# filrg/attackFL

Measured on AMD Instinct MI355X. Metric: FL rounds/sec (whole node) + test-acc, TransformerModel/ICU, 8 clients, higher is better.
Workload: dtype bf16; 1 GPU; model=TransformerModel, global_batch=1024, seq_len=1, parallelism=fl8-clients-over-1-ranks, clients=8, local_epochs=5, rows_per_client=12000-15000, mode=fedavg, trainer=fused

## Files before the change

### csrc/kernels/tf2.hip

```cpp
#include "common.h"
#include "kernels.h"
#include "tf_common.h"
#include "fused_common.h"
#define ONCHIP_NO_AGPR
#include "onchip.h"

using namespace tf;

namespace t2 {

using namespace oc;



constexpr int LDDN = 24 * 2, LDVO = LD64 + 16;
constexpr int B_IMG_D = 0;
constexpr int B_IMG_V = B_IMG_D + 64 * LDDN;
constexpr int B_IMG_O = B_IMG_V + 64 * LDVO;
constexpr int B_IMG_F1 = B_IMG_O + 64 * LDVO;
constexpr int B_IMG_F2 = B_IMG_F1 + 16 * LD64;
constexpr int B_H0 = B_IMG_F2 + 64 * LD32;
constexpr int B_A = B_H0 + 16384;
constexpr int B_X1N = B_A + 16384;
constexpr int B_DF3 = B_X1N + 16384;
constexpr int B_DO = B_DF3 + 16384;
constexpr int B_DV = B_DO + 16384;
constexpr int B_DZ0 = B_DV + 16384;
constexpr int B_XIN = B_DZ0 + 16384;
constexpr int B_F2 = B_XIN + 4096;
constexpr int B_DF0 = B_F2 + 4096;
constexpr int B_NVEC = 648;
constexpr int B_VEC = B_DF0 + 4096;
constexpr int B_NLN = 6 * 64;
constexpr int B_DBL = B_VEC + B_NVEC * 4;
constexpr int B_DBL_BYTES = B_NLN * 8;
constexpr int B_MISC = B_DBL + B_DBL_BYTES;
constexpr int B_CNT_A = B_MISC + 32;
constexpr int B_CNT_B = B_MISC + 36;
constexpr int B_CNT_C = B_MISC + 40;
constexpr int B_TOTAL = B_MISC + 64;
enum { VS_DB = 0, VS_VB, VS_OB, VS_G1, VS_B1, VS_F2B, VS_G2, VS_B2, VS_G3, VS_B3 };
constexpr int VS_F1B = 640;

#ifndef TF2_HLD1
#define TF2_HLD1 (LD128 + 16)
#endif
#ifndef TF2_HLD2
#define TF2_HLD2 (LD64 + 16)
#endif
constexpr int HLD1 = TF2_HLD1, HLD2 = TF2_HLD2;
constexpr int H_IMG_W1 = 0;
constexpr int H_IMG_W2 = H_IMG_W1 + 64 * HLD1;
constexpr int H_CAT = H_IMG_W2 + 32 * HLD2;
constexpr int H_A1 = H_CAT + 32768;
constexpr int H_DZ1 = H_A1 + 16384;
constexpr int H_DZ2 = H_DZ1 + 16384;
constexpr int H_NVEC = 132;
constexpr int H_VEC = H_DZ2 + 8192;
constexpr int H_PART = H_VEC + H_NVEC * 4;
constexpr int H_LOSS = H_PART + 8 * H_NVEC * 4;
constexpr int H_CNT = H_LOSS + 64;
constexpr int H_TOTAL = H_CNT + 16;
enum { HV_B1 = 0, HV_B2 = 64, HV_WO = 96, HV_BO = 128 };

constexpr int SMEM_CORE = B_TOTAL > H_TOTAL ? B_TOTAL : H_TOTAL;
// ... 19 lines not shown
  float s;
  const int f = colsum64(x, lane, s);
  lds_addq(smem + B_DBL, 64 * k + f, s);
}
__host__ __device__ constexpr int ln_seg(int k) { return k < 2 ? VS_G1 + k : VS_G2 + (k - 2); }
static_assert(ln_seg(0) == VS_G1 && ln_seg(1) == VS_B1 && ln_seg(2) == VS_G2 && ln_seg(3) == VS_B2 &&
              ln_seg(4) == VS_G3 && ln_seg(5) == VS_B3, "DBL order");

__device__ __forceinline__ uint32_t mask16(uint32_t key, uint32_t layer, int r, int g, uint32_t thr) {
  uint32_t m = 0;
#pragma unroll
  for (int t = 0; t < 4; ++t) {
#pragma unroll
    for (int h = 0; h < 2; ++h) {
      const uint32_t x = hash3(key, layer, (uint32_t)r, (uint32_t)(8 * t + 2 * g + h));
      m |= ((x & 0xFFFFu) >= thr ? 1u : 0u) << (4 * t + 2 * h);
      m |= ((x >> 16) >= thr ? 1u : 0u) << (4 * t + 2 * h + 1);
    }
  }
  return m;
}


#ifdef TF2_STAMPS
struct Stamp {
  bool on = false;
  int who = 0;
  uchar* smem = nullptr;
  __device__ __forceinline__ void operator()(int id, int tid) {
    if (!on) return;
    const uint64_t now = __builtin_amdgcn_s_memrealtime();
    if (tid == who) {
      LDS_AS uint64_t* t = (LDS_AS uint64_t*)(smem + ST_OFF);
      t[id] += now - t[ST_N - 1];
      t[ST_N - 1] = now;
    }
  }
};
#else
struct Stamp {
  __device__ __forceinline__ void operator()(int, int) {}
};
#endif

enum { ABL_U3 = 1, ABL_UADAM = 2, ABL_UDW = 4, ABL_COLSUM = 8, ABL_HEADUPD = 16, ABL_U1 = 32 };
#if defined(TF2_STAMPS) && defined(TF2_ABL)
#define ABL(K, b) ((TF2_ABL & (b)) != 0)
#else
#define ABL(K, b) false
#endif



#ifndef TF2_NO_PRIO
__device__ __forceinline__ void prio_hi() { __builtin_amdgcn_s_setprio(2); }
__device__ __forceinline__ void prio_lo() { __builtin_amdgcn_s_setprio(0); }
#else
__device__ __forceinline__ void prio_hi() {}
__device__ __forceinline__ void prio_lo() {}
#endif

template <int BR>
struct BrK {
  static constexpr BrOff o = BR == 0 ? OV : OL;
  static constexpr int din = BR == 0 ? D_V : D_L;
  static constexpr int xoff = BR == 0 ? 0 : D_V;
  static constexpr Mat MV{o.inproj_w + 128 * 64, 64, 64, B_IMG_V, LDVO};
  static constexpr Mat MO{o.out_w, 64, 64, B_IMG_O, LDVO};
  static __device__ __forceinline__ Mat vo(bool lo) {
    return Mat{lo ? MV.off : MO.off, 64, 64, lo ? B_IMG_V : B_IMG_O, LDVO};
  }
  static __device__ __forceinline__ int vec_param(int e) {
    if (e >= VS_F1B) return e - VS_F1B < FF ? o.ff0_b + (e - VS_F1B) : -1;
    const int s = e >> 6, i = e & 63;
    const int b = s == 0 ? o.dense_b : s == 1 ? o.inproj_b + 128 : s == 2 ? o.out_b : s == 3 ? o.ln1_w
                : s == 4 ? o.ln1_b : s == 5 ? o.ff3_b : s == 6 ? o.ln2_w : s == 7 ? o.ln2_b : s == 8 ? o.bn_w : o.bn_b;
    return b + i;
  }
};

struct Saved {
  uint32_t xh1[8], xh2[8], gp[8];
  float rstd1, rstd2;
  uint32_t m1, m2, matt;
  float gk[4];
};
__device__ __forceinline__ void save16(uint32_t (&d)[8], const float (&x)[16]) {
#pragma unroll
  for (int k = 0; k < 8; ++k) d[k] = pk2(x[2 * k], x[2 * k + 1]);
}
__device__ __forceinline__ void load16(float (&x)[16], const uint32_t (&d)[8]) {
#pragma unroll
  for (int k = 0; k < 8; ++k) {
    x[2 * k] = __uint_as_float(d[k] << 16);
    x[2 * k + 1] = __uint_as_float(d[k] & 0xFFFF0000u);
  }
}

constexpr int NCMP = 2;
struct BrState {
  VS cmp[NCMP];
};
__device__ __forceinline__ int vec_entry(int wave, int lane, int h) {
  const int w4 = wave & 3, g = lane >> 4, i16 = lane & 15;
  const bool lead = wave < 4;
  if (h == 0) {
    if (wave >= 2) return ln_seg(wave - 2) * 64 + lane;
    return wave == 0 && g == 0 && VS_F1B + i16 < B_NVEC ? VS_F1B + i16 : -1;
  }
  if (g < 2) return (w4 & 1) == 0 ? (lead ? VS_OB : VS_VB) * 64 + 16 * (2 * (w4 >> 1) + g) + i16 : -1;
  return lead ? (g == 2 ? VS_F2B : VS_DB) * 64 + 16 * w4 + i16 : -1;
}
__device__ __forceinline__ bool vec_real(int e) { return e >= 0 && e < VS_F1B + FF; }

template <int BR>
__device__ __forceinline__ void br_masks(uint32_t key, int r, int g, uint32_t& mk0, uint32_t& mk1) {
  const uint32_t ha = hash3(key, 8 * BR + L_ATT, r, 0), hb = hash3(key, 8 * BR + L_ATT, r, 1);
  const uint32_t matt = ((ha & 0xFFFFu) >= THR_P01 ? 1u : 0u) | ((ha >> 16) >= THR_P01 ? 2u : 0u) |
                        ((hb & 0xFFFFu) >= THR_P01 ? 4u : 0u) | ((hb >> 16) >= THR_P01 ? 8u : 0u);
  const uint32_t m1 = mask16(key, 8 * BR + L_D1, r, g, THR_P01), m2 = mask16(key, 8 * BR + L_D2, r, g, THR_P01);
  uint32_t kf = 0u;
  if (g < 2) {
    const uint32_t hd[2] = {hash3(key, 8 * BR + L_DF, r, 2 * g), hash3(key, 8 * BR + L_DF, r, 2 * g + 1)};
#pragma unroll
    for (int i = 0; i < 4; ++i) {
      const uint32_t u = (hd[i >> 1] >> ((i & 1) << 4)) & 0xFFFFu;
      kf |= (4 * g + i < FF && u >= THR_P01 ? 1u : 0u) << i;
    }
  }
  mk0 = m1 | (m2 << 16);
  mk1 = matt | (kf << 4);
}

template <int BR>
__device__ __forceinline__ void br_forward(uchar* smem, const float (&xin)[4], uint32_t mk0, uint32_t mk1, Saved& sv,
                                           u32x4 (&outp)[2], int lane, int wave) {
  using B = BrK<BR>;
  opq(lane, wave);
  const int g = lane >> 4, r = 16 * wave + (lane & 15);
  const uchar* vg = lane_vec(smem + B_VEC, g);
  st4<TK16>(smem + B_XIN, r, g, xin);
  float h0[16];
  sb();
  {
    const s4v bx = bfrag4(xin);
    f4v acc[4];
#pragma unroll
    for (int T = 0; T < 4; ++T)
      acc[T] = mma16(*(const LDS_AS s4v*)(smem + B_IMG_D + (16 * T + (lane & 15)) * LDDN + 8 * (lane >> 4)), bx, Z4);
    float bd[16], gp[16];
    vec16g(bd, vg + VS_DB * 256);
#pragma unroll
    for (int t = 0; t < 4; ++t)
#pragma unroll
      for (int i = 0; i < 4; i += 2) {
        gf2v g2;
        const gf2v y = gelu2(gf2v{acc[t][i] + bd[4 * t + i], acc[t][i + 1] + bd[4 * t + i + 1]}, g2);
        h0[4 * t + i] = y[0];
        h0[4 * t + i + 1] = y[1];
        gp[4 * t + i] = g2[0];
        gp[4 * t + i + 1] = g2[1];
      }
    save16(sv.gp, gp);
#pragma unroll
    for (int t = 0; t < 4; ++t) st4<TK64>(smem + B_H0, r, 4 * t + g, h0 + 4 * t);
  }
  float a[16];
  sb();
  {
    const s8v b0 = bfrag(h0, 0), b1 = bfrag(h0, 1);
    f4v acc[4];
#pragma unroll
    for (int T = 0; T < 4; ++T) {
      acc[T] = mma(wfrag(smem + B_IMG_V, LDVO, T, 0, lane), b0, Z4);
      acc[T] = mma(wfrag(smem + B_IMG_V, LDVO, T, 1, lane), b1, acc[T]);
    }
    sv.matt = mk1 & 0xFu;
    float bv[16];
    vec16g(bv, vg + VS_VB * 256);
#pragma unroll
    for (int t = 0; t < 4; ++t) {
      const float m = keepf(INV_K01, sv.matt, t);
#pragma unroll
      for (int i = 0; i < 4; ++i) a[4 * t + i] = (acc[t][i] + bv[4 * t + i]) * m;
    }
#pragma unroll
    for (int t = 0; t < 4; ++t) st4<TK64>(smem + B_A, r, 4 * t + g, a + 4 * t);
  }
  float x1n[16];
  sb();
  {
    const s8v b0 = bfrag(a, 0), b1 = bfrag(a, 1);
    f4v acc[4];
#pragma unroll
    for (int T = 0; T < 4; ++T) {
      acc[T] = mma(wfrag(smem + B_IMG_O, LDVO, T, 0, lane), b0, Z4);
      acc[T] = mma(wfrag(smem + B_IMG_O, LDVO, T, 1, lane), b1, acc[T]);
    }
    sv.m1 = mk0 & 0xFFFFu;
    float bo[16];
    vec16g(bo, vg + VS_OB * 256);
    float x1[16];
#pragma unroll
    for (int t = 0; t < 4; ++t)
#pragma unroll
      for (int i = 0; i < 4; ++i) {
        const int j = 4 * t + i;
        x1[j] = h0[j] + keepf((acc[t][i] + bo[j]) * INV_K01, sv.m1, j);
      }
    sv.rstd1 = ln_fwd2(x1);
    save16(sv.xh1, x1);
    float gm[16], bt[16];
    vec16g(gm, vg + VS_G1 * 256);
    vec16g(bt, vg + VS_B1 * 256);
    affine2(x1n, x1, gm, bt);
#pragma unroll
    for (int t = 0; t < 4; ++t) st4<TK64>(smem + B_X1N, r, 4 * t + g, x1n + 4 * t);
  }
  float f2v[4];
  sb();
  {
    f4v acc = mma(wfrag(smem + B_IMG_F1, LD64, 0, 0, lane), bfrag(x1n, 0), Z4);
    acc = mma(wfrag(smem + B_IMG_F1, LD64, 0, 1, lane), bfrag(x1n, 1), acc);
    const f4v bf = g < 2 ? *(const LDS_AS f4v*)(vg + VS_F1B * 4) : Z4;
#pragma unroll
    for (int i = 0; i < 4; ++i) {
      float gp;
      const float gl = gelu_and_grad(acc[i] + bf[i], gp);
      f2v[i] = keepf(gl * INV_K01, mk1, 4 + i);
      sv.gk[i] = keepf(gp * INV_K01, mk1, 4 + i);
    }
    st4<TK16>(smem + B_F2, r, g, f2v);
  }
  sb();
  {
    const s4v bf = bfrag4(f2v);
    f4v acc[4];
#pragma unroll
    for (int T = 0; T < 4; ++T) acc[T] = mma16(wfrag4(smem + B_IMG_F2, LD32, T, lane), bf, Z4);
    sv.m2 = mk0 >> 16;
    float b3[16];
    vec16g(b3, vg + VS_F2B * 256);
    float x2[16];
#pragma unroll
    for (int t = 0; t < 4; ++t)
#pragma unroll
      for (int i = 0; i < 4; ++i) {
        const int j = 4 * t + i;
        x2[j] = x1n[j] + keepf((acc[t][i] + b3[j]) * INV_K01, sv.m2, j);
      }
    sv.rstd2 = ln_fwd2(x2);
    save16(sv.xh2, x2);
    float gm[16], bt[16];
    vec16g(gm, vg + VS_G2 * 256);
    vec16g(bt, vg + VS_B2 * 256);
    affine2(x2, x2, gm, bt);
    ln_fwd2(x2);
    vec16g(gm, vg + VS_G3 * 256);
    vec16g(bt, vg + VS_B3 * 256);
    affine2(x2, x2, gm, bt);
    pack16(x2, outp);
  }
}

struct BwdPre {
  float xh3[16], rstd3;
  s8v f3[2];
};
__device__ __forceinline__ void br_bwd_pre(const uchar* smem, const Saved& sv, BwdPre& bp, int lane) {
  const uchar* vg = lane_vec(smem + B_VEC, lane >> 4);
  float gm[16], bt[16];
  load16(bp.xh3, sv.xh2);
  vec16g(gm, vg + VS_G2 * 256);
  vec16g(bt, vg + VS_B2 * 256);
  affine2(bp.xh3, bp.xh3, gm, bt);
  bp.rstd3 = ln_fwd2(bp.xh3);
#pragma unroll
  for (int j = 0; j < 16; ++j) asm volatile("" : "+v"(bp.xh3[j]));
  asm volatile("" : "+v"(bp.rstd3));
  bp.f3[0] = wtfrag<true>(smem + B_IMG_F2, LD32, 0, 0, lane);
  bp.f3[1] = wtfrag<true>(smem + B_IMG_F2, LD32, 0, 1, lane);
  asm volatile("" : "+v"(bp.f3[0]), "+v"(bp.f3[1]));
}

template <int BR>
__device__ __forceinline__ void br_backward(uchar* smem, const float (&dout)[16], const Saved& sv, const BwdPre& bp,
                                            const AdamK& K, int lane, int wave) {
  opq(lane, wave);
  const int g = lane >> 4, r = 16 * wave + (lane & 15);
  const uchar* vg = lane_vec(smem + B_VEC, g);
  float dr2[16];
  sb();
  {
    float gm[16], t[16], dx[16], xh[16];
#pragma unroll
    for (int j = 0; j < 16; ++j) xh[j] = bp.xh3[j];
    const float rstd3 = bp.rstd3;
#pragma unroll
    for (int j = 0; j < 16; ++j) t[j] = dout[j] * xh[j];
    if (!ABL(K, ABL_COLSUM)) ln_colsum(smem, 4, t, lane);
    if (!ABL(K, ABL_COLSUM)) ln_colsum(smem, 5, dout, lane);
    vec16g(gm, vg + VS_G3 * 256);
    ln_bwd2(dx, dout, xh, rstd3, gm);
    load16(xh, sv.xh2);
#pragma unroll
    for (int j = 0; j < 16; ++j) t[j] = dx[j] * xh[j];
    if (!ABL(K, ABL_COLSUM)) ln_colsum(smem, 2, t, lane);
    if (!ABL(K, ABL_COLSUM)) ln_colsum(smem, 3, dx, lane);
    vec16g(gm, vg + VS_G2 * 256);
    ln_bwd2(dr2, dx, xh, sv.rstd2, gm);
  }
  float df0[4];
  sb();
  {
    float d3[16];
#pragma unroll
    for (int j = 0; j < 16; ++j) d3[j] = keepf(dr2[j] * INV_K01, sv.m2, j);
#pragma unroll
    for (int t = 0; t < 4; ++t) st4<TK64>(smem + B_DF3, r, 4 * t + g, d3 + 4 * t);
    f4v acc = mma(bp.f3[0], bfrag(d3, 0), Z4);
    acc = mma(bp.f3[1], bfrag(d3, 1), acc);
#pragma unroll
    for (int i = 0; i < 4; ++i) df0[i] = acc[i] * sv.gk[i];
    st4<TK16>(smem + B_DF0, r, g, df0);
  }
  lds_signal(smem, B_CNT_C, lane);
  float dr1[16];
  sb();
  {
    const s4v bd = bfrag4(df0);
    float dx[16];
#pragma unroll
    for (int T = 0; T < 4; ++T) {
      const f4v acc = mma16(wtfrag4(smem + B_IMG_F1, LD64, T, lane), bd, Z4);
#pragma unroll
      for (int i = 0; i < 4; ++i) dx[4 * T + i] = acc[i] + dr2[4 * T + i];
    }
    float t[16], gm[16], xh[16];
    load16(xh, sv.xh1);
#pragma unroll
    for (int j = 0; j < 16; ++j) t[j] = dx[j] * xh[j];
    if (!ABL(K, ABL_COLSUM)) ln_colsum(smem, 0, t, lane);
    if (!ABL(K, ABL_COLSUM)) ln_colsum(smem, 1, dx, lane);
    vec16g(gm, vg + VS_G1 * 256);
    ln_bwd2(dr1, dx, xh, sv.rstd1, gm);
  }
  float dv[16];
  sb();
  {
    float dO[16];
#pragma unroll
    for (int j = 0; j < 16; ++j) dO[j] = keepf(dr1[j] * INV_K01, sv.m1, j);
#pragma unroll
    for (int t = 0; t < 4; ++t) st4<TK64>(smem + B_DO, r, 4 * t + g, dO + 4 * t);
    const s8v b0 = bfrag(dO, 0), b1 = bfrag(dO, 1);
#pragma unroll
    for (int T = 0; T < 4; ++T) {
      f4v acc = mma(wtfrag<true>(smem + B_IMG_O, LDVO, T, 0, lane), b0, Z4);
      acc = mma(wtfrag<true>(smem + B_IMG_O, LDVO, T, 1, lane), b1, acc);
      const float m = keepf(INV_K01, sv.matt, T);
#pragma unroll
      for (int i = 0; i < 4; ++i) dv[4 * T + i] = acc[i] * m;
    }
#pragma unroll
    for (int t = 0; t < 4; ++t) st4<TK64>(smem + B_DV, r, 4 * t + g, dv + 4 * t);
  }
  lds_signal(smem, B_CNT_A, lane);
  sb();
  {
    const s8v b0 = bfrag(dv, 0), b1 = bfrag(dv, 1);
    float dz[16], gp[16];
    load16(gp, sv.gp);
#pragma unroll
    for (int T = 0; T < 4; ++T) {
      f4v acc = mma(wtfrag<true>(smem + B_IMG_V, LDVO, T, 0, lane), b0, Z4);
      acc = mma(wtfrag<true>(smem + B_IMG_V, LDVO, T, 1, lane), b1, acc);
#pragma unroll
      for (int i = 0; i < 4; ++i) dz[4 * T + i] = (acc[i] + dr1[4 * T + i]) * gp[4 * T + i];
    }
#pragma unroll
    for (int t = 0; t < 4; ++t) st4<TK64>(smem + B_DZ0, r, 4 * t + g, dz + 4 * t);
  }
  lds_signal(smem, B_CNT_B, lane);
}


template <int BR>
__device__ __forceinline__ int cmp_param(int e) {
  return vec_real(e) ? BrK<BR>::vec_param(e) : -1;
}

__device__ __forceinline__ f4v unit_ld(__amdgpu_buffer_rsrc_t rm, int ui, int j, int lane) {
  return __builtin_bit_cast(f4v, __builtin_amdgcn_raw_buffer_load_b128(rm, (int)BR_UNITS + ((ui * 12 + j) * 64 + lane) * 16,
                                                                        0, 16));
}
__device__ __forceinline__ void unit_st(__amdgpu_buffer_rsrc_t rm, int ui, int j, int lane, f4v v) {
  __builtin_amdgcn_raw_buffer_store_b128(__builtin_bit_cast(u32x4, v), rm, (int)BR_UNITS + ((ui * 12 + j) * 64 + lane) * 16,
                                         0, 0);
  store_guard();
}
__device__ __forceinline__ void unit_adam(f4v (&U)[12], const f4v (&acc)[2][2], const AdamK& K) {
  float p[16], mm[16], vv[16], g[16], den[16];
#pragma unroll
  for (int t = 0; t < 4; ++t)
#pragma unroll
    for (int i = 0; i < 4; ++i) {
      mm[4 * t + i] = U[t][i];
      vv[4 * t + i] = U[4 + t][i];
      p[4 * t + i] = U[8 + t][i];
      g[4 * t + i] = acc[t >> 1][t & 1][i];
    }
#pragma unroll
  for (int e = 0; e < 16; ++e) {
    const float mk = mm[e] * K.keep;
    mm[e] = mk + K.c1 * (g[e] - mk);
    vv[e] = fk::B2 * vv[e] + (1.f - fk::B2) * g[e] * g[e];
  }
#pragma unroll
  for (int e = 0; e < 16; ++e) den[e] = __builtin_amdgcn_sqrtf(vv[e]);
#pragma unroll
  for (int e = 0; e < 16; ++e) den[e] = __builtin_amdgcn_rcpf(den[e] * K.rsqrt_bc2 + K.eps);
#pragma unroll
  for (int e = 0; e < 16; ++e) p[e] -= K.lr_bc1 * mm[e] * den[e];
#pragma unroll
  for (int t = 0; t < 4; ++t)
#pragma unroll
    for (int i = 0; i < 4; ++i) {
      U[t][i] = mm[4 * t + i];
      U[4 + t][i] = vv[4 * t + i];
      U[8 + t][i] = p[4 * t + i];
    }
}
__device__ __forceinline__ void unit_img(uchar* smem, const Mat& M, int Ta, int Tb, int lane, const u32x2v (&w)[4]) {
  const int i16 = lane & 15, g4 = 4 * (lane >> 4);
#pragma unroll
  for (int t = 0; t < 4; ++t)
    *(LDS_AS u32x2v*)(smem + M.img + (16 * (Tb + (t & 1)) + i16) * M.ld + pcol(16 * (Ta + (t >> 1)) + g4) * 2) = w[t];
}
__device__ __forceinline__ void unit_pack(const f4v (&U)[12], u32x2v (&w)[4]) {
#pragma unroll
  for (int t = 0; t < 4; ++t) w[t] = u32x2v{pk2(U[8 + t][0], U[8 + t][1]), pk2(U[8 + t][2], U[8 + t][3])};
}
__device__ __forceinline__ void unit_dw(const uchar* X, const uchar* DY, int Ta, int Tb, int lane, bool bias,
                                        f4v (&acc)[2][2], f4v (&bs)[2]) {
#pragma unroll
  for (int a = 0; a < 2; ++a)
#pragma unroll
    for (int b = 0; b < 2; ++b) acc[a][b] = Z4;
  bs[0] = bs[1] = Z4;
  uint32_t o1 = 0x3F803F80u;
  asm volatile("" : "+s"(o1));
  const s8v one = __builtin_bit_cast(s8v, u32x4{o1, o1, o1, o1});
#pragma unroll
  for (int s = 0; s < 4; ++s) {
    const s8v x0 = tfrag<TK64>(X, 32 * s, Ta, lane), x1 = tfrag<TK64>(X, 32 * s, Ta + 1, lane);
    const s8v y0 = tfrag<TK64>(DY, 32 * s, Tb, lane), y1 = tfrag<TK64>(DY, 32 * s, Tb + 1, lane);
    acc[0][0] = mma(x0, y0, acc[0][0]);
    acc[0][1] = mma(x0, y1, acc[0][1]);
    acc[1][0] = mma(x1, y0, acc[1][0]);
    acc[1][1] = mma(x1, y1, acc[1][1]);
    if (bias) {
      bs[0] = mma(one, y0, bs[0]);
      bs[1] = mma(one, y1, bs[1]);
    }
  }
}

__device__ __forceinline__ f4v smu_ld(__amdgpu_buffer_rsrc_t rm, int w4, int j, int lane) {
  return __builtin_bit_cast(f4v, __builtin_amdgcn_raw_buffer_load_b128(rm, (int)BR_SMALL + ((w4 * 9 + j) * 64 + lane) * 16,
                                                                        0, 16));
}
__device__ __forceinline__ void smu_st(__amdgpu_buffer_rsrc_t rm, int w4, int j, int lane, f4v v) {
  __builtin_amdgcn_raw_buffer_store_b128(__builtin_bit_cast(u32x4, v), rm, (int)BR_SMALL + ((w4 * 9 + j) * 64 + lane) * 16,
                                         0, 0);
  store_guard();
}
template <int BR>
__device__ __forceinline__ void smu_elem(int s, int w4, int lane, int i, int& pi, int& img) {
  using B = BrK<BR>;
  constexpr int din = BrK<BR>::din;
  const int g = lane >> 4, i16 = lane & 15;
  if (s == 0) {
    const int n = 16 * w4 + i16, k = 4 * g + i;
    pi = k < din ? B::o.dense_w + n * din + k : -1;
    img = B_IMG_D + n * LDDN + k * 2;
  } else if (s == 1) {
    const int n = 16 * w4 + i16, k = 4 * g + i;
    pi = k < FF ? B::o.ff3_w + n * FF + k : -1;
    img = B_IMG_F2 + n * LD32 + pcol(k) * 2;
  } else {
    const int n = i16, k = 16 * w4 + 4 * g + i;
    pi = n < FF ? B::o.ff0_w + n * 64 + k : -1;
    img = B_IMG_F1 + n * LD64 + pcol(k) * 2;
  }
}
__device__ __forceinline__ void smu_adam(f4v (&S)[9], const f4v (&gs)[3], const AdamK& K) {
  float p[12], mm[12], vv[12], g[12], den[12];
#pragma unroll
  for (int s = 0; s < 3; ++s)
#pragma unroll
    for (int i = 0; i < 4; ++i) {
      mm[4 * s + i] = S[s][i];
      vv[4 * s + i] = S[3 + s][i];
      p[4 * s + i] = S[6 + s][i];
      g[4 * s + i] = gs[s][i];
    }
#pragma unroll
  for (int e = 0; e < 12; ++e) {
    const float mk = mm[e] * K.keep;
    mm[e] = mk + K.c1 * (g[e] - mk);
    vv[e] = fk::B2 * vv[e] + (1.f - fk::B2) * g[e] * g[e];
  }
#pragma unroll
  for (int e = 0; e < 12; ++e) den[e] = __builtin_amdgcn_sqrtf(vv[e]);
#pragma unroll
  for (int e = 0; e < 12; ++e) den[e] = __builtin_amdgcn_rcpf(den[e] * K.rsqrt_bc2 + K.eps);
#pragma unroll
  for (int e = 0; e < 12; ++e) p[e] -= K.lr_bc1 * mm[e] * den[e];
#pragma unroll
  for (int s = 0; s < 3; ++s)
#pragma unroll
    for (int i = 0; i < 4; ++i) {
      S[s][i] = mm[4 * s + i];
      S[3 + s][i] = vv[4 * s + i];
      S[6 + s][i] = p[4 * s + i];
    }
}
template <int BR>
__device__ __forceinline__ void smu_img(uchar* smem, const f4v (&S)[9], int w4, int lane) {
#pragma unroll
  for (int s = 0; s < 3; ++s) {
    int pi, img;
    smu_elem<BR>(s, w4, lane, 0, pi, img);
    *(LDS_AS u32x2v*)(smem + img) = u32x2v{pk2(S[6 + s][0], S[6 + s][1]), pk2(S[6 + s][2], S[6 + s][3])};
  }
}

template <int N>
__device__ __forceinline__ void vec_adam(VS (&pa)[N], float (&m)[N], float (&v)[N], const float (&g)[N], float (&pn)[N],
                                         const AdamK& K) {
#pragma clang fp contract(off)
  float den[N];
#pragma unroll
  for (int i = 0; i < N; ++i) {
    pn[i] = ar(pa[i].p);
    const float mk = m[i] * K.keep;
    m[i] = __builtin_fmaf(K.c1, g[i] - mk, mk);
    const float t = (1.f - fk::B2) * g[i], u = fk::B2 * v[i];
    v[i] = __builtin_fmaf(g[i], t, u);
  }
#pragma unroll
  for (int i = 0; i < N; ++i) den[i] = __builtin_amdgcn_sqrtf(v[i]);
#pragma unroll
  for (int i = 0; i < N; ++i) den[i] = __builtin_amdgcn_rcpf(__builtin_fmaf(K.rsqrt_bc2, den[i], K.eps));
#pragma unroll
  for (int i = 0; i < N; ++i) {
    const float lm = K.lr_bc1 * m[i];
    pn[i] = __builtin_fmaf(-lm, den[i], pn[i]);
    pa[i].p = aw(pn[i]);
  }
}

template <int BR>
__device__ __forceinline__ bool br_update(uchar* smem, BrState& st, const AdamK& K, int lane, int wave, int tid, int step,
                                          __amdgpu_buffer_rsrc_t rm, Stamp& stp, gu32* tmo) {
  using B = BrK<BR>;
  opq(lane, wave);
  asm volatile("" : "+v"(tid));
  const int w4 = wave & 3, g = lane >> 4;
  const bool lead = wave < 4;
  const uint32_t all = 8u * (uint32_t)step;
  LDS_AS uint32_t* abort_w = ldsu(smem, B_MISC);
  const int Ta = 2 * (w4 & 1), Tb = 2 * (w4 >> 1);
  const bool do_bias = (w4 & 1) == 0;
  f4v bsu[2] = {Z4, Z4};
  f4v cmom;
  f4v as = Z4, bd = Z4, a3 = Z4, af1 = Z4, b3 = Z4, b1 = Z4;
  const int ui = 2 * w4 + (lead ? 0 : 1);
  f4v U[12];
#pragma unroll
  for (int j = 0; j < 12; ++j) U[j] = unit_ld(rm, ui, j, lane);
  uint32_t o1 = 0x3F803F80u;
  asm volatile("" : "+s"(o1));
  const s8v one = __builtin_bit_cast(s8v, u32x4{o1, o1, o1, o1});
  if (lead) {
    prio_lo();
    if (!lds_wait(smem, B_CNT_C, all)) {
      if (lane == 0) __hip_atomic_store(tmo, 1u, __ATOMIC_RELAXED, __HIP_MEMORY_SCOPE_AGENT);
      return false;
    }
#pragma unroll
    for (int s = 0; s < (ABL(K, ABL_U1) ? 0 : 4); ++s) {
      const s8v y3 = tfrag<TK64>(smem + B_DF3, 32 * s, w4, lane), y1 = tfrag<TK16>(smem + B_DF0, 32 * s, 0, lane);
      a3 = mma(tfrag<TK16>(smem + B_F2, 32 * s, 0, lane), y3, a3);
      af1 = mma(tfrag<TK64>(smem + B_X1N, 32 * s, w4, lane), y1, af1);
      b3 = mma(one, y3, b3);
      if (wave == 0) b1 = mma(one, y1, b1);
    }
    if (!lds_wait(smem, B_CNT_A, all)) {
      if (lane == 0) __hip_atomic_store(tmo, 1u, __ATOMIC_RELAXED, __HIP_MEMORY_SCOPE_AGENT);
      return false;
    }
    prio_hi();
  } else {
    if (!lds_wait(smem, B_CNT_A, all)) {
      if (lane == 0) __hip_atomic_store(tmo, 1u, __ATOMIC_RELAXED, __HIP_MEMORY_SCOPE_AGENT);
      return false;
    }
  }
  {
    uint32_t any = 0;
#pragma unroll
    for (int i = 0; i < 8; ++i) any |= abort_w[i];
    if (any) return false;
  }
  stp(4, tid);
  {
    f4v acc[2][2];
    if (!ABL(K, ABL_UDW))
      unit_dw(smem + (lead ? B_A : B_H0), smem + (lead ? B_DO : B_DV), Ta, Tb, lane, do_bias, acc, bsu);
    if (!ABL(K, ABL_UADAM)) unit_adam(U, acc, K);
    u32x2v w[4];
    unit_pack(U, w);
    cmom = mom_ld(rm, 0, tid);
    if (!lead && !lds_wait(smem, B_CNT_B, all)) {
      if (lane == 0) __hip_atomic_store(tmo, 1u, __ATOMIC_RELAXED, __HIP_MEMORY_SCOPE_AGENT);
      return false;
    }
    unit_img(smem, B::vo(!lead), Ta, Tb, lane, w);
#pragma unroll
    for (int j = 0; j < 12; ++j) unit_st(rm, ui, j, lane, U[j]);
  }
  if (lead) {
    f4v S[9];
#pragma unroll
    for (int j = 0; j < 9; ++j) S[j] = smu_ld(rm, w4, j, lane);
    if (!lds_wait(smem, B_CNT_B, all)) {
      if (lane == 0) __hip_atomic_store(tmo, 1u, __ATOMIC_RELAXED, __HIP_MEMORY_SCOPE_AGENT);
      return false;
    }
#pragma unroll
    for (int s = 0; s < (ABL(K, ABL_U1) ? 0 : 4); ++s) {
      const s8v yd = tfrag<TK64>(smem + B_DZ0, 32 * s, w4, lane);
      as = mma(tfrag<TK16>(smem + B_XIN, 32 * s, 0, lane), yd, as);
      bd = mma(one, yd, bd);
    }
    const f4v gs3[3] = {as, a3, af1};
    if (!ABL(K, ABL_U3)) smu_adam(S, gs3, K);
    smu_img<BR>(smem, S, w4, lane);
#pragma unroll
    for (int j = 0; j < 9; ++j) smu_st(rm, w4, j, lane, S[j]);
  }
  stp(5, tid);
  prio_hi();
  float gr[NCMP];
  gr[0] = b1[0];
  if (wave >= 2) {
    LDS_AS double* q = (LDS_AS double*)(smem + B_DBL) + 64 * (wave - 2) + lane;
    gr[0] = lds_getq(smem + B_DBL, 64 * (wave - 2) + lane);
    *q = 0.0;
  }
  gr[1] = g == 0 ? bsu[0][0] : g == 1 ? bsu[1][0] : g == 2 ? b3[0] : bd[0];
  float mm[NCMP] = {cmom[0], cmom[1]}, vv[NCMP] = {cmom[2], cmom[3]};
  if (!ABL(K, ABL_U3)) {
    float pn[NCMP];
    vec_adam<NCMP>(st.cmp, mm, vv, gr, pn, K);
#pragma unroll
    for (int h = 0; h < NCMP; ++h) {
      const int e = vec_entry(wave, lane, h);
      if (vec_real(e)) ldsf(smem, B_VEC)[e] = pn[h];
    }
  }
  mom_st(rm, 0, tid, f4v{mm[0], mm[1], vv[0], vv[1]});
  return true;
}

__device__ __forceinline__ void mom_zero(__amdgpu_buffer_rsrc_t rm, int tid) {
#pragma unroll
  for (int k = 0; k < MOM_SLOTS; ++k) mom_st(rm, k, tid, Z4);
}

template <int BR>
__device__ __forceinline__ void br_init(uchar* smem, BrState& st, const float* P, __amdgpu_buffer_rsrc_t rm, int lane,
                                        int wave, int tid) {
  using B = BrK<BR>;
#pragma unroll
  for (int k = 0; k < CMP_SLOTS; ++k) mom_st(rm, k, tid, Z4);
  {
    const int w4 = wave & 3, u = wave >> 2, Ta = 2 * (w4 & 1), Tb = 2 * (w4 >> 1);
    const Mat M = B::vo(u == 1);
    const int i16 = lane & 15, g4 = 4 * (lane >> 4);
#pragma unroll
    for (int t = 0; t < 4; ++t) {
      const int n = 16 * (Tb + (t & 1)) + i16, k0 = 16 * (Ta + (t >> 1)) + g4;
      const float* src = P + M.off + n * M.k_real + k0;
      const f4v p = {src[0], src[1], src[2], src[3]};
      unit_st(rm, 2 * w4 + u, t, lane, Z4);
      unit_st(rm, 2 * w4 + u, 4 + t, lane, Z4);
      unit_st(rm, 2 * w4 + u, 8 + t, lane, p);
      *(LDS_AS u32x2v*)(smem + M.img + n * M.ld + pcol(k0) * 2) = u32x2v{pk2(p[0], p[1]), pk2(p[2], p[3])};
    }
  }
  if (wave < 4) {
    f4v S[9];
#pragma unroll
    for (int s = 0; s < 3; ++s) {
      S[s] = S[3 + s] = Z4;
#pragma unroll
      for (int i = 0; i < 4; ++i) {
        int pi, img;
        smu_elem<BR>(s, wave, lane, i, pi, img);
        S[6 + s][i] = pi >= 0 ? P[pi] : 0.f;
      }
    }
    smu_img<BR>(smem, S, wave, lane);
#pragma unroll
    for (int j = 0; j < 9; ++j) smu_st(rm, wave, j, lane, S[j]);
  }
#pragma unroll
  for (int h = 0; h < NCMP; ++h) {
    const int e = vec_entry(wave, lane, h);
    float p0 = 0.f;
    if (e >= 0) {
      const int pi = cmp_param<BR>(e);
      p0 = pi >= 0 ? P[pi] : 0.f;
      ldsf(smem, B_VEC)[e] = p0;
// ... 78 lines not shown
  if (stp.on && tid == 0)
    for (int i = 0; i < ST_N - 1; ++i) a.stamps[i] = *(LDS_AS uint64_t*)(smem + ST_OFF + 8 * i);
#endif
  (void)stp; (void)a; (void)smem; (void)tid;
}

template <int BR>
__device__ __forceinline__ void branch_main(const AflTfTrainArgs& a, int cid, uchar* smem) {
  const int tid = threadIdx.x, lane = tid & 63, wave = __builtin_amdgcn_readfirstlane(tid >> 6), g = lane >> 4;
  float* P = a.params + (long)cid * NPARAM;
  uchar* ws = (uchar*)(a.ws + (long)cid * a.ws_stride);
  gu32* sync = (gu32*)(a.sync + (long)cid * AFL_TF2H_SYNC_WORDS);
  const __amdgpu_buffer_rsrc_t rg = gr_rsrc(sync);
  for (int i = tid; i < SMEM / 4; i += NTH) ldsf(smem, 0)[i] = 0.f;
  __syncthreads();
  BrState st;
  const __amdgpu_buffer_rsrc_t rm = rsrc(ws + WS_MOM + MOM_WG_BYTES + BR * BR_WG_BYTES);
  br_init<BR>(smem, st, P, rm, lane, wave, tid);
  asm volatile("s_waitcnt vmcnt(0)" ::: "memory");
  __syncthreads();
  Stamp stp;
  stamp_init(stp, a, smem);

  const int nd = a.nd[cid], BS = a.batch, E = a.E;
  const uint32_t seed = a.seeds[cid];
  LDS_AS uint32_t* abort_w = ldsu(smem, B_MISC);
  int step = 0;
  bool failed = false;
  Walk w{0, 0};
  float xin[4];
  bool more = walk_valid(w, nd, BS, E);
  if (more) load_x<BR>(xin, a, cid, w, lane, wave);
  float mka0, mka1;
  {
    uint32_t m0, m1;
    br_masks<BR>(afl_hash32(seed, 1u), 16 * wave + (lane & 15), g, m0, m1);
    mka0 = awu(m0);
    mka1 = awu(m1);
  }
  while (more) {
    ++step;
    const AdamK K = adam_k(a, step);
    Saved sv;
    u32x4 outp[2];
    prio_hi();
    asm volatile(";MARK fwd");
#ifndef TF2_NO_FWD
    br_forward<BR>(smem, xin, aru(mka0), aru(mka1), sv, outp, lane, wave);
#else
    sv = Saved{}; outp[0] = u32x4{0,0,0,0}; outp[1] = outp[0];
#endif
    asm volatile(";MARK fwd_end");
    stp(0, tid);
    gr_put(rg, gr_off(0, BR, wave, lane), outp, (uint32_t)step);
    prio_lo();
    w.b0 += BS;
    more = walk_valid(w, nd, BS, E);
    if (more) load_x<BR>(xin, a, cid, w, lane, wave);
    {
      uint32_t m0, m1;
      br_masks<BR>(afl_hash32(seed, (uint32_t)(step + 1)), 16 * wave + (lane & 15), g, m0, m1);
      mka0 = awu(m0);
      mka1 = awu(m1);
    }
    BwdPre bp;
    sb();
    br_bwd_pre(smem, sv, bp, lane);
    sb();
    stp(1, tid);
    u32x4 du[2];
    const int go[1] = {gr_off(1, BR, wave, lane)};
    const uint32_t fv = gr_get<1>(rg, go, du, (uint32_t)step, 1, sync + XF_TMO, lane);
    prio_hi();
    stp(2, tid);
    if (fv == 0xFFFFFFFFu) {
      if (lane == 0) abort_w[wave] = 1u;
      lds_signal(smem, B_CNT_C, lane);
      lds_signal(smem, B_CNT_A, lane);
      lds_signal(smem, B_CNT_B, lane);
      failed = true;
      break;
    }
    float dout[16];
    unpack16(du, dout);
    if (lane == 0) abort_w[wave] = fv & 1u;
#ifndef TF2_NO_BWD
    asm volatile(";MARK bwd");
    br_backward<BR>(smem, dout, sv, bp, K, lane, wave);
    asm volatile(";MARK bwd_end");
    stp(3, tid);
#else
    for (int j = 0; j < 16; ++j) asm volatile("" :: "v"(dout[j]));
    lds_signal(smem, B_CNT_C, lane);
    lds_signal(smem, B_CNT_A, lane);
    lds_signal(smem, B_CNT_B, lane);
#endif
    asm volatile(";MARK upd");
    const bool upd_ok = br_update<BR>(smem, st, K, lane, wave, tid, step, rm, stp, sync + XF_TMO);
    asm volatile(";MARK upd_end");
    if (!upd_ok) {
      failed = true;
      break;
    }
    stp(7, tid);
    lds_bar();
    stp(8, tid);
  }
  (void)failed;
  stamp_fini(stp, a, smem, tid);
  br_fini<BR>(st, P, rm, lane, wave, tid);
}

constexpr Mat HW1{FC1_W, 64, 128, H_IMG_W1, HLD1};
constexpr Mat HW2{FC2_W, 32, 64, H_IMG_W2, HLD2};
__device__ __forceinline__ int hvec_param(int e) {
  return e < 64 ? FC1_B + e : e < 96 ? FC2_B + (e - 64) : e < 128 ? OUT_W + (e - 96) : e == 128 ? OUT_B : -1;
}
struct HdState {
  TS blk[4];
  TS t2;
  VS vec;
};

constexpr int NWG = 4;
constexpr int EX_SLOTS = 5;
constexpr int EX_BASE = 2 * GR_DIR_BYTES;
static_assert(EX_BASE == AFL_GR_WORDS * 4 && 2 * 8 * EX_SLOTS * 1024 == AFL_EX_WORDS, "export slots follow the hand-off slots");
__device__ __forceinline__ int ex_off(int parity, int tile, int k, int lane) {
  return EX_BASE + ((parity * 8 + tile) * EX_SLOTS + k) * 4096 + lane * 16;
}

__device__ __forceinline__ void head_main(const AflTfTrainArgs& a, int cid, uchar* smem, int half) {
  const int tid = threadIdx.x, lane = tid & 63, wave = __builtin_amdgcn_readfirstlane(tid >> 6), g = lane >> 4;
  const bool crit = wave < 4;
  const int tile = crit ? 4 * half + wave : 4 * (1 - half) + (wave - 4);
  const int r = 16 * tile + (lane & 15);
  float* P = a.params + (long)cid * NPARAM;
  uchar* ws = (uchar*)(a.ws + (long)cid * a.ws_stride);
  gu32* sync = (gu32*)(a.sync + (long)cid * AFL_TF2H_SYNC_WORDS);
  const __amdgpu_buffer_rsrc_t rg = gr_rsrc(sync);
  for (int i = tid; i < SMEM / 4; i += NTH) ldsf(smem, 0)[i] = 0.f;
  __syncthreads();
  HdState st;
  Stamp stp;
  const __amdgpu_buffer_rsrc_t rm = rsrc(ws + (half == 0 ? WS_MOM : WS_MOM2));
  mom_zero(rm, tid);
  {
    const int Ta = 2 * (wave & 3), Tb = 2 * (wave >> 2);
#pragma unroll
    for (int x = 0; x < 2; ++x)
#pragma unroll
      for (int y = 0; y < 2; ++y) tile_load(st.blk[2 * x + y], HW1, Ta + x, Tb + y, lane, P, smem);
    tile_load(st.t2, HW2, wave & 3, wave >> 2, lane, P, smem);
    float p0 = 0.f;
    if (tid < H_NVEC) {
      const int pi = hvec_param(tid);
      p0 = pi >= 0 ? P[pi] : 0.f;
      ldsf(smem, H_VEC)[tid] = p0;
    }
// ... 441 lines not shown
```

Measured before the change: 129.4 rounds/s.

## Prefetch weight fragments, fold vector Adam into unit Adam, use SGPR-offset exchange

Forward and backward passes now load the next layer's MMA weight fragments from LDS one stage early and pin them in registers, so LDS latency overlaps the current stage's math. The per-parameter vector Adam update is merged into the matrix-unit and small-unit Adam loops, so it runs alongside them and its momentum load is issued earlier. The cross-workgroup gradient put/get now uses a scalar base offset with a per-lane voffset. The extra live fragments raise VGPR pressure, which may cost occupancy or cause spills.

```diff
diff --git a/csrc/kernels/tf2.hip b/csrc/kernels/tf2.hip
--- a/csrc/kernels/tf2.hip
+++ b/csrc/kernels/tf2.hip
@@ -10,7 +10,6 @@
 namespace t2 {
 
 using namespace oc;
-
 
 
 constexpr int LDDN = 24 * 2, LDVO = LD64 + 16;
@@ -136,6 +135,45 @@
 
 
 
+__device__ __forceinline__ int gr_soff(int dir, int src, int wave) { return dir * GR_DIR_BYTES + (src * 8 + wave) * 4096; }
+__device__ __forceinline__ void gr_put_s(__amdgpu_buffer_rsrc_t rg, int soff, int lane16, const u32x4 (&u)[2],
+                                         uint32_t tag) {
+#pragma unroll
+  for (int k = 0; k < 4; ++k) {
+    const int j = 2 * (k & 1);
+    __builtin_amdgcn_raw_buffer_store_b128(u32x4{u[k >> 1][j], tag, u[k >> 1][j + 1], tag}, rg, lane16 + k * 1024, soff, 16);
+    store_guard();
+  }
+}
+template <int S>
+__device__ __forceinline__ uint32_t gr_get_s(__amdgpu_buffer_rsrc_t rg, const int (&soff)[S], int lane16,
+                                             u32x4 (&out)[2 * S], uint32_t want, int shift, gu32* tmo, int lane) {
+  for (long spins = 0;; ++spins) {
+    u32x4 v[4 * S];
+#pragma unroll
+    for (int s = 0; s < S; ++s)
+#pragma unroll
+      for (int k = 0; k < 4; ++k)
+        v[4 * s + k] = __builtin_amdgcn_raw_buffer_load_b128(rg, lane16 + k * 1024, soff[s], 16);
+    bool ok = true;
+#pragma unroll
+    for (int i = 0; i < 4 * S; ++i) ok = ok && (v[i][1] >> shift) == want && (v[i][3] >> shift) == want;
+    if (__builtin_amdgcn_ballot_w64(!ok) == 0) {
+#pragma unroll
+      for (int s = 0; s < S; ++s) {
+        out[2 * s] = u32x4{v[4 * s][0], v[4 * s][2], v[4 * s + 1][0], v[4 * s + 1][2]};
+        out[2 * s + 1] = u32x4{v[4 * s + 2][0], v[4 * s + 2][2], v[4 * s + 3][0], v[4 * s + 3][2]};
+      }
+      return __builtin_amdgcn_readfirstlane(v[0][1]);
+    }
+    if (spins > fk::XWG_MAX_SPINS) {
+      if (lane == 0) __hip_atomic_store(tmo, 1u, __ATOMIC_RELAXED, __HIP_MEMORY_SCOPE_AGENT);
+      return 0xFFFFFFFFu;
+    }
+    __builtin_amdgcn_s_sleep(1);
+  }
+}
+
 #ifndef TF2_NO_PRIO
 __device__ __forceinline__ void prio_hi() { __builtin_amdgcn_s_setprio(2); }
 __device__ __forceinline__ void prio_lo() { __builtin_amdgcn_s_setprio(0); }
@@ -216,6 +254,12 @@
   mk1 = matt | (kf << 4);
 }
 
+template <int N, class V>
+__device__ __forceinline__ void pin(V (&f)[N]) {
+#pragma unroll
+  for (int i = 0; i < N; ++i) asm volatile("" : "+v"(f[i]));
+}
+
 template <int BR>
 __device__ __forceinline__ void br_forward(uchar* smem, const float (&xin)[4], uint32_t mk0, uint32_t mk1, Saved& sv,
                                            u32x4 (&outp)[2], int lane, int wave) {
@@ -225,13 +269,22 @@
   const uchar* vg = lane_vec(smem + B_VEC, g);
   st4<TK16>(smem + B_XIN, r, g, xin);
   float h0[16];
+  s8v pfv[4], pfo[4], pf1[2];
+  s4v pf3[4];
   sb();
   {
     const s4v bx = bfrag4(xin);
     f4v acc[4];
+    s4v wd[4];
 #pragma unroll
     for (int T = 0; T < 4; ++T)
-      acc[T] = mma16(*(const LDS_AS s4v*)(smem + B_IMG_D + (16 * T + (lane & 15)) * LDDN + 8 * (lane >> 4)), bx, Z4);
+      wd[T] = *(const LDS_AS s4v*)(smem + B_IMG_D + (16 * T + (lane & 15)) * LDDN + 8 * (lane >> 4));
+    sb();
+#pragma unroll
+    for (int T = 0; T < 4; ++T) pfv[T] = wfrag(smem + B_IMG_V, LDVO, T, 0, lane);
+    sb();
+#pragma unroll
+    for (int T = 0; T < 4; ++T) acc[T] = mma16(wd[T], bx, Z4);
     float bd[16], gp[16];
     vec16g(bd, vg + VS_DB * 256);
 #pragma unroll
@@ -248,16 +301,23 @@
     save16(sv.gp, gp);
 #pragma unroll
     for (int t = 0; t < 4; ++t) st4<TK64>(smem + B_H0, r, 4 * t + g, h0 + 4 * t);
+    pin(pfv);
   }
   float a[16];
   sb();
   {
+    s8v w1[4];
+#pragma unroll
+    for (int T = 0; T < 4; ++T) w1[T] = wfrag(smem + B_IMG_V, LDVO, T, 1, lane);
+#pragma unroll
+    for (int T = 0; T < 4; ++T) pfo[T] = wfrag(smem + B_IMG_O, LDVO, T, 0, lane);
+    sb();
     const s8v b0 = bfrag(h0, 0), b1 = bfrag(h0, 1);
     f4v acc[4];
 #pragma unroll
     for (int T = 0; T < 4; ++T) {
-      acc[T] = mma(wfrag(smem + B_IMG_V, LDVO, T, 0, lane), b0, Z4);
-      acc[T] = mma(wfrag(smem + B_IMG_V, LDVO, T, 1, lane), b1, acc[T]);
+      acc[T] = mma(pfv[T], b0, Z4);
+      acc[T] = mma(w1[T], b1, acc[T]);
     }
     sv.matt = mk1 & 0xFu;
     float bv[16];
@@ -270,16 +330,23 @@
     }
 #pragma unroll
     for (int t = 0; t < 4; ++t) st4<TK64>(smem + B_A, r, 4 * t + g, a + 4 * t);
+    pin(pfo);
   }
   float x1n[16];
   sb();
   {
+    s8v w1[4];
+#pragma unroll
+    for (int T = 0; T < 4; ++T) w1[T] = wfrag(smem + B_IMG_O, LDVO, T, 1, lane);
+    pf1[0] = wfrag(smem + B_IMG_F1, LD64, 0, 0, lane);
+    pf1[1] = wfrag(smem + B_IMG_F1, LD64, 0, 1, lane);
+    sb();
     const s8v b0 = bfrag(a, 0), b1 = bfrag(a, 1);
     f4v acc[4];
 #pragma unroll
     for (int T = 0; T < 4; ++T) {
-      acc[T] = mma(wfrag(smem + B_IMG_O, LDVO, T, 0, lane), b0, Z4);
-      acc[T] = mma(wfrag(smem + B_IMG_O, LDVO, T, 1, lane), b1, acc[T]);
+      acc[T] = mma(pfo[T], b0, Z4);
+      acc[T] = mma(w1[T], b1, acc[T]);
     }
     sv.m1 = mk0 & 0xFFFFu;
     float bo[16];
@@ -300,12 +367,16 @@
     affine2(x1n, x1, gm, bt);
 #pragma unroll
     for (int t = 0; t < 4; ++t) st4<TK64>(smem + B_X1N, r, 4 * t + g, x1n + 4 * t);
+    pin(pf1);
   }
   float f2v[4];
   sb();
   {
-    f4v acc = mma(wfrag(smem + B_IMG_F1, LD64, 0, 0, lane), bfrag(x1n, 0), Z4);
-    acc = mma(wfrag(smem + B_IMG_F1, LD64, 0, 1, lane), bfrag(x1n, 1), acc);
+#pragma unroll
+    for (int T = 0; T < 4; ++T) pf3[T] = wfrag4(smem + B_IMG_F2, LD32, T, lane);
+    sb();
+    f4v acc = mma(pf1[0], bfrag(x1n, 0), Z4);
+    acc = mma(pf1[1], bfrag(x1n, 1), acc);
     const f4v bf = g < 2 ? *(const LDS_AS f4v*)(vg + VS_F1B * 4) : Z4;
 #pragma unroll
     for (int i = 0; i < 4; ++i) {
@@ -315,13 +386,14 @@
       sv.gk[i] = keepf(gp * INV_K01, mk1, 4 + i);
     }
     st4<TK16>(smem + B_F2, r, g, f2v);
+    pin(pf3);
   }
   sb();
   {
     const s4v bf = bfrag4(f2v);
     f4v acc[4];
 #pragma unroll
-    for (int T = 0; T < 4; ++T) acc[T] = mma16(wfrag4(smem + B_IMG_F2, LD32, T, lane), bf, Z4);
+    for (int T = 0; T < 4; ++T) acc[T] = mma16(pf3[T], bf, Z4);
     sv.m2 = mk0 >> 16;
     float b3[16];
     vec16g(b3, vg + VS_F2B * 256);
@@ -395,8 +467,13 @@
     ln_bwd2(dr2, dx, xh, sv.rstd2, gm);
   }
   float df0[4];
+  s4v pt1[4];
+  s8v pto[4], ptv[4];
   sb();
   {
+#pragma unroll
+    for (int T = 0; T < 4; ++T) pt1[T] = wtfrag4(smem + B_IMG_F1, LD64, T, lane);
+    sb();
     float d3[16];
 #pragma unroll
     for (int j = 0; j < 16; ++j) d3[j] = keepf(dr2[j] * INV_K01, sv.m2, j);
@@ -407,16 +484,20 @@
 #pragma unroll
     for (int i = 0; i < 4; ++i) df0[i] = acc[i] * sv.gk[i];
     st4<TK16>(smem + B_DF0, r, g, df0);
+    pin(pt1);
   }
   lds_signal(smem, B_CNT_C, lane);
   float dr1[16];
   sb();
   {
+#pragma unroll
+    for (int T = 0; T < 4; ++T) pto[T] = wtfrag<true>(smem + B_IMG_O, LDVO, T, 0, lane);
+    sb();
     const s4v bd = bfrag4(df0);
     float dx[16];
 #pragma unroll
     for (int T = 0; T < 4; ++T) {
-      const f4v acc = mma16(wtfrag4(smem + B_IMG_F1, LD64, T, lane), bd, Z4);
+      const f4v acc = mma16(pt1[T], bd, Z4);
 #pragma unroll
       for (int i = 0; i < 4; ++i) dx[4 * T + i] = acc[i] + dr2[4 * T + i];
     }
@@ -428,10 +509,14 @@
     if (!ABL(K, ABL_COLSUM)) ln_colsum(smem, 1, dx, lane);
     vec16g(gm, vg + VS_G1 * 256);
     ln_bwd2(dr1, dx, xh, sv.rstd1, gm);
+    pin(pto);
   }
   float dv[16];
   sb();
   {
+#pragma unroll
+    for (int T = 0; T < 4; ++T) ptv[T] = wtfrag<true>(smem + B_IMG_V, LDVO, T, 0, lane);
+    sb();
     float dO[16];
 #pragma unroll
     for (int j = 0; j < 16; ++j) dO[j] = keepf(dr1[j] * INV_K01, sv.m1, j);
@@ -440,7 +525,7 @@
     const s8v b0 = bfrag(dO, 0), b1 = bfrag(dO, 1);
 #pragma unroll
     for (int T = 0; T < 4; ++T) {
-      f4v acc = mma(wtfrag<true>(smem + B_IMG_O, LDVO, T, 0, lane), b0, Z4);
+      f4v acc = mma(pto[T], b0, Z4);
       acc = mma(wtfrag<true>(smem + B_IMG_O, LDVO, T, 1, lane), b1, acc);
       const float m = keepf(INV_K01, sv.matt, T);
 #pragma unroll
@@ -448,6 +533,7 @@
     }
 #pragma unroll
     for (int t = 0; t < 4; ++t) st4<TK64>(smem + B_DV, r, 4 * t + g, dv + 4 * t);
+    pin(ptv);
   }
   lds_signal(smem, B_CNT_A, lane);
   sb();
@@ -457,7 +543,7 @@
     load16(gp, sv.gp);
 #pragma unroll
     for (int T = 0; T < 4; ++T) {
-      f4v acc = mma(wtfrag<true>(smem + B_IMG_V, LDVO, T, 0, lane), b0, Z4);
+      f4v acc = mma(ptv[T], b0, Z4);
       acc = mma(wtfrag<true>(smem + B_IMG_V, LDVO, T, 1, lane), b1, acc);
 #pragma unroll
       for (int i = 0; i < 4; ++i) dz[4 * T + i] = (acc[i] + dr1[4 * T + i]) * gp[4 * T + i];
@@ -483,8 +569,43 @@
                                          0, 0);
   store_guard();
 }
-__device__ __forceinline__ void unit_adam(f4v (&U)[12], const f4v (&acc)[2][2], const AdamK& K) {
-  float p[16], mm[16], vv[16], g[16], den[16];
+struct VecAd {
+  float m[NCMP], v[NCMP], g[NCMP], pn[NCMP];
+};
+template <int N, int NA, int NV>
+__device__ __forceinline__ void adam_pinned(float (&p)[N], float (&mm)[N], float (&vv)[N], const float (&g)[N],
+                                            const AdamK& K) {
+#pragma clang fp contract(off)
+  float den[N];
+#pragma unroll
+  for (int e = 0; e < N; ++e) {
+    const float mk = mm[e] * K.keep;
+    const float d = e < N - NV ? __builtin_fmaf(-K.keep, mm[e], g[e]) : g[e] - mk;
+    mm[e] = __builtin_fmaf(K.c1, d, mk);
+    const float t = (1.f - fk::B2) * g[e];
+    if (e < NA) {
+      const float t2 = g[e] * t;
+      vv[e] = __builtin_fmaf(fk::B2, vv[e], t2);
+    } else {
+      const float u = fk::B2 * vv[e];
+      vv[e] = __builtin_fmaf(g[e], t, u);
+    }
+  }
+#pragma unroll
+  for (int e = 0; e < N; ++e) den[e] = __builtin_amdgcn_sqrtf(vv[e]);
+#pragma unroll
+  for (int e = 0; e < N; ++e) den[e] = __builtin_amdgcn_rcpf(__builtin_fmaf(K.rsqrt_bc2, den[e], K.eps));
+#pragma unroll
+  for (int e = 0; e < N; ++e) {
+    const float lm = K.lr_bc1 * mm[e];
+    p[e] = __builtin_fmaf(-lm, den[e], p[e]);
+  }
+}
+template <int NV>
+__device__ __forceinline__ void unit_adam(f4v (&U)[12], const f4v (&acc)[2][2], const AdamK& K, VS (&pa)[NCMP],
+                                          VecAd& x) {
+  static_assert(NV == 0 || NV == NCMP, "all of the thread's vector entries or none");
+  float p[16 + NV], mm[16 + NV], vv[16 + NV], g[16 + NV];
 #pragma unroll
   for (int t = 0; t < 4; ++t)
 #pragma unroll
@@ -495,17 +616,13 @@
       g[4 * t + i] = acc[t >> 1][t & 1][i];
     }
 #pragma unroll
-  for (int e = 0; e < 16; ++e) {
-    const float mk = mm[e] * K.keep;
-    mm[e] = mk + K.c1 * (g[e] - mk);
-    vv[e] = fk::B2 * vv[e] + (1.f - fk::B2) * g[e] * g[e];
-  }
-#pragma unroll
-  for (int e = 0; e < 16; ++e) den[e] = __builtin_amdgcn_sqrtf(vv[e]);
-#pragma unroll
-  for (int e = 0; e < 16; ++e) den[e] = __builtin_amdgcn_rcpf(den[e] * K.rsqrt_bc2 + K.eps);
-#pragma unroll
-  for (int e = 0; e < 16; ++e) p[e] -= K.lr_bc1 * mm[e] * den[e];
+  for (int h = 0; h < NV; ++h) {
+    mm[16 + h] = x.m[h];
+    vv[16 + h] = x.v[h];
+    p[16 + h] = ar(pa[h].p);
+    g[16 + h] = x.g[h];
+  }
+  adam_pinned<16 + NV, 16, NV>(p, mm, vv, g, K);
 #pragma unroll
   for (int t = 0; t < 4; ++t)
 #pragma unroll
@@ -514,6 +631,13 @@
       U[4 + t][i] = vv[4 * t + i];
       U[8 + t][i] = p[4 * t + i];
     }
+#pragma unroll
+  for (int h = 0; h < NV; ++h) {
+    x.m[h] = mm[16 + h];
+    x.v[h] = vv[16 + h];
+    x.pn[h] = p[16 + h];
+    pa[h].p = aw(p[16 + h]);
+  }
 }
 __device__ __forceinline__ void unit_img(uchar* smem, const Mat& M, int Ta, int Tb, int lane, const u32x2v (&w)[4]) {
   const int i16 = lane & 15, g4 = 4 * (lane >> 4);
@@ -578,8 +702,10 @@
     img = B_IMG_F1 + n * LD64 + pcol(k) * 2;
   }
 }
-__device__ __forceinline__ void smu_adam(f4v (&S)[9], const f4v (&gs)[3], const AdamK& K) {
-  float p[12], mm[12], vv[12], g[12], den[12];
+template <int NV>
+__device__ __forceinline__ void smu_adam(f4v (&S)[9], const f4v (&gs)[3], const AdamK& K, VS (&pa)[NCMP], VecAd& x) {
+  static_assert(NV == 0 || NV == NCMP, "all of the thread's vector entries or none");
+  float p[12 + NV], mm[12 + NV], vv[12 + NV], g[12 + NV];
 #pragma unroll
   for (int s = 0; s < 3; ++s)
 #pragma unroll
@@ -590,17 +716,13 @@
       g[4 * s + i] = gs[s][i];
     }
 #pragma unroll
-  for (int e = 0; e < 12; ++e) {
-    const float mk = mm[e] * K.keep;
-    mm[e] = mk + K.c1 * (g[e] - mk);
-    vv[e] = fk::B2 * vv[e] + (1.f - fk::B2) * g[e] * g[e];
-  }
-#pragma unroll
-  for (int e = 0; e < 12; ++e) den[e] = __builtin_amdgcn_sqrtf(vv[e]);
-#pragma unroll
-  for (int e = 0; e < 12; ++e) den[e] = __builtin_amdgcn_rcpf(den[e] * K.rsqrt_bc2 + K.eps);
-#pragma unroll
-  for (int e = 0; e < 12; ++e) p[e] -= K.lr_bc1 * mm[e] * den[e];
+  for (int h = 0; h < NV; ++h) {
+    mm[12 + h] = x.m[h];
+    vv[12 + h] = x.v[h];
+    p[12 + h] = ar(pa[h].p);
+    g[12 + h] = x.g[h];
+  }
+  adam_pinned<12 + NV, 4, NV>(p, mm, vv, g, K);
 #pragma unroll
   for (int s = 0; s < 3; ++s)
 #pragma unroll
@@ -609,6 +731,13 @@
       S[3 + s][i] = vv[4 * s + i];
       S[6 + s][i] = p[4 * s + i];
     }
+#pragma unroll
+  for (int h = 0; h < NV; ++h) {
+    x.m[h] = mm[12 + h];
+    x.v[h] = vv[12 + h];
+    x.pn[h] = p[12 + h];
+    pa[h].p = aw(p[12 + h]);
+  }
 }
 template <int BR>
 __device__ __forceinline__ void smu_img(uchar* smem, const f4v (&S)[9], int w4, int lane) {
@@ -617,31 +746,6 @@
     int pi, img;
     smu_elem<BR>(s, w4, lane, 0, pi, img);
     *(LDS_AS u32x2v*)(smem + img) = u32x2v{pk2(S[6 + s][0], S[6 + s][1]), pk2(S[6 + s][2], S[6 + s][3])};
-  }
-}
-
-template <int N>
-__device__ __forceinline__ void vec_adam(VS (&pa)[N], float (&m)[N], float (&v)[N], const float (&g)[N], float (&pn)[N],
-                                         const AdamK& K) {
-#pragma clang fp contract(off)
-  float den[N];
-#pragma unroll
-  for (int i = 0; i < N; ++i) {
-    pn[i] = ar(pa[i].p);
-    const float mk = m[i] * K.keep;
-    m[i] = __builtin_fmaf(K.c1, g[i] - mk, mk);
-    const float t = (1.f - fk::B2) * g[i], u = fk::B2 * v[i];
-    v[i] = __builtin_fmaf(g[i], t, u);
-  }
-#pragma unroll
-  for (int i = 0; i < N; ++i) den[i] = __builtin_amdgcn_sqrtf(v[i]);
-#pragma unroll
-  for (int i = 0; i < N; ++i) den[i] = __builtin_amdgcn_rcpf(__builtin_fmaf(K.rsqrt_bc2, den[i], K.eps));
-#pragma unroll
-  for (int i = 0; i < N; ++i) {
-    const float lm = K.lr_bc1 * m[i];
-    pn[i] = __builtin_fmaf(-lm, den[i], pn[i]);
-    pa[i].p = aw(pn[i]);
   }
 }
 
@@ -658,12 +762,12 @@
   const int Ta = 2 * (w4 & 1), Tb = 2 * (w4 >> 1);
   const bool do_bias = (w4 & 1) == 0;
   f4v bsu[2] = {Z4, Z4};
-  f4v cmom;
   f4v as = Z4, bd = Z4, a3 = Z4, af1 = Z4, b3 = Z4, b1 = Z4;
   const int ui = 2 * w4 + (lead ? 0 : 1);
   f4v U[12];
 #pragma unroll
   for (int j = 0; j < 12; ++j) U[j] = unit_ld(rm, ui, j, lane);
+  const f4v cmom = mom_ld(rm, 0, tid);
   uint32_t o1 = 0x3F803F80u;
   asm volatile("" : "+s"(o1));
   const s8v one = __builtin_bit_cast(s8v, u32x4{o1, o1, o1, o1});
@@ -699,21 +803,45 @@
     if (any) return false;
   }
   stp(4, tid);
+  VecAd x;
+  x.g[0] = b1[0];
+  if (wave >= 2) {
+    LDS_AS double* q = (LDS_AS double*)(smem + B_DBL) + 64 * (wave - 2) + lane;
+    x.g[0] = lds_getq(smem + B_DBL, 64 * (wave - 2) + lane);
+    *q = 0.0;
+  }
+  auto vec_in = [&]() {
+    x.g[1] = g == 0 ? bsu[0][0] : g == 1 ? bsu[1][0] : g == 2 ? b3[0] : bd[0];
+    x.m[0] = cmom[0], x.m[1] = cmom[1], x.v[0] = cmom[2], x.v[1] = cmom[3];
+  };
+  auto vec_out = [&]() {
+#pragma unroll
+    for (int h = 0; h < NCMP; ++h) {
+      const int e = vec_entry(wave, lane, h);
+      if (vec_real(e)) ldsf(smem, B_VEC)[e] = x.pn[h];
+    }
+  };
   {
     f4v acc[2][2];
     if (!ABL(K, ABL_UDW))
       unit_dw(smem + (lead ? B_A : B_H0), smem + (lead ? B_DO : B_DV), Ta, Tb, lane, do_bias, acc, bsu);
-    if (!ABL(K, ABL_UADAM)) unit_adam(U, acc, K);
+    if (!lead) {
+      vec_in();
+      if (!ABL(K, ABL_UADAM)) unit_adam<NCMP>(U, acc, K, st.cmp, x);
+    } else {
+      if (!ABL(K, ABL_UADAM)) unit_adam<0>(U, acc, K, st.cmp, x);
+    }
     u32x2v w[4];
     unit_pack(U, w);
-    cmom = mom_ld(rm, 0, tid);
     if (!lead && !lds_wait(smem, B_CNT_B, all)) {
       if (lane == 0) __hip_atomic_store(tmo, 1u, __ATOMIC_RELAXED, __HIP_MEMORY_SCOPE_AGENT);
       return false;
     }
     unit_img(smem, B::vo(!lead), Ta, Tb, lane, w);
+    if (!lead && !ABL(K, ABL_UADAM)) vec_out();
 #pragma unroll
     for (int j = 0; j < 12; ++j) unit_st(rm, ui, j, lane, U[j]);
+    if (!lead) mom_st(rm, 0, tid, f4v{x.m[0], x.m[1], x.v[0], x.v[1]});
   }
   if (lead) {
     f4v S[9];
@@ -730,32 +858,14 @@
       bd = mma(one, yd, bd);
     }
     const f4v gs3[3] = {as, a3, af1};
-    if (!ABL(K, ABL_U3)) smu_adam(S, gs3, K);
+    vec_in();
+    if (!ABL(K, ABL_U3)) smu_adam<NCMP>(S, gs3, K, st.cmp, x);
     smu_img<BR>(smem, S, w4, lane);
+    if (!ABL(K, ABL_U3)) vec_out();
 #pragma unroll
     for (int j = 0; j < 9; ++j) smu_st(rm, w4, j, lane, S[j]);
-  }
-  stp(5, tid);
-  prio_hi();
-  float gr[NCMP];
-  gr[0] = b1[0];
-  if (wave >= 2) {
-    LDS_AS double* q = (LDS_AS double*)(smem + B_DBL) + 64 * (wave - 2) + lane;
-    gr[0] = lds_getq(smem + B_DBL, 64 * (wave - 2) + lane);
-    *q = 0.0;
-  }
-  gr[1] = g == 0 ? bsu[0][0] : g == 1 ? bsu[1][0] : g == 2 ? b3[0] : bd[0];
-  float mm[NCMP] = {cmom[0], cmom[1]}, vv[NCMP] = {cmom[2], cmom[3]};
-  if (!ABL(K, ABL_U3)) {
-    float pn[NCMP];
-    vec_adam<NCMP>(st.cmp, mm, vv, gr, pn, K);
-#pragma unroll
-    for (int h = 0; h < NCMP; ++h) {
-      const int e = vec_entry(wave, lane, h);
-      if (vec_real(e)) ldsf(smem, B_VEC)[e] = pn[h];
-    }
-  }
-  mom_st(rm, 0, tid, f4v{mm[0], mm[1], vv[0], vv[1]});
+    mom_st(rm, 0, tid, f4v{x.m[0], x.m[1], x.v[0], x.v[1]});
+  }
   return true;
 }
 
@@ -940,7 +1050,7 @@
 #endif
     asm volatile(";MARK fwd_end");
     stp(0, tid);
-    gr_put(rg, gr_off(0, BR, wave, lane), outp, (uint32_t)step);
+    gr_put_s(rg, gr_soff(0, BR, wave), 16 * lane, outp, (uint32_t)step);
     prio_lo();
     w.b0 += BS;
     more = walk_valid(w, nd, BS, E);
@@ -957,8 +1067,8 @@
     sb();
     stp(1, tid);
     u32x4 du[2];
-    const int go[1] = {gr_off(1, BR, wave, lane)};
-    const uint32_t fv = gr_get<1>(rg, go, du, (uint32_t)step, 1, sync + XF_TMO, lane);
+    const int go[1] = {gr_soff(1, BR, wave)};
+    const uint32_t fv = gr_get_s<1>(rg, go, 16 * lane, du, (uint32_t)step, 1, sync + XF_TMO, lane);
     prio_hi();
     stp(2, tid);
     if (fv == 0xFFFFFFFFu) {
@@ -990,9 +1100,9 @@
       failed = true;
       break;
     }
-    stp(7, tid);
+    stp(5, tid);
     lds_bar();
-    stp(8, tid);
+    stp(6, tid);
   }
   (void)failed;
   stamp_fini(stp, a, smem, tid);
```

After: 133.6 rounds/s, median of 6. 1.03x the previous value.
